# RManLuo/MAMDR

Hardware: AMD Instinct MI355X
Metric: domain-steps/sec (higher is better)
Workload: dtype f32; 1 GPU; mlp_meta_mamdr Taobao-10 bs=1024 (frozen pretrained tables); global_batch=1024, domains=10, step_definition=one MAMDR meta-epoch (DN + DR phases, all outer updates), parallelism=single GPU

## Files before the change

### mamdr_amd/csrc/fused_kernels.hip

```cpp
#include <hip/hip_ext.h>

#include "mamdr_kernels.h"
#include "wgrad_adam_deal.h"

namespace mamdr {

constexpr int FZ_THREADS = 512;
constexpr int FZ_WAVES = 8;
constexpr int FZ_RING = 32;
static_assert(FZ_SBLK == DM_PARTS && FZ_DEAL_EMB == EMB && FZ_DEAL_H1 == H1 && FZ_DEAL_H2 == H2 && FZ_DEAL_H3 == H3,
              "wgrad_adam_deal.h deals the tower of mamdr_device.h");
static_assert(FZ_OUTB == 2 && FZ_OWN == FZ_SBLK + FZ_TILES + FZ_OUTB, "two output-unit workgroups of 32 columns of h3");
__host__ __device__ constexpr int fz_own_wgs(bool with_loss) { return FZ_OWN + (with_loss ? 1 : 0); }
__constant__ const FzDealTable c_fz_deal = fz_deal_table_make();

#define FZSTAMP(k) MAMDR_STAMP(MAMDR_CYCLES, a.stamps && threadIdx.x == 0, a.stamps[blockIdx.x * 8 + (k)])
#define FZREAL(k) MAMDR_STAMP(MAMDR_REALTIME, a.stamps && threadIdx.x == 0, a.stamps[blockIdx.x * 8 + (k)])

__device__ __forceinline__ void fz_store(const FusedArgs& a, int e, float p, float m, float v) {
    if (a.optimizer == 2) {
        a.m[e] = m;
        return;
    }
    if (a.optimizer == 0) {
// ... 111 lines not shown
    return s > FZ_LDS_TILE ? s : FZ_LDS_TILE;
}

__device__ __forceinline__ void fz_tile_body(const FusedArgs& a, const FzTile ft, float* lds) {
    const int tid = threadIdx.x, lane = tid & 63, j = lane & 15, kq = lane >> 4;
    const int w = __builtin_amdgcn_readfirstlane(tid >> 6);
    const int gemm = ft.gemm, ablk = ft.ablk, bblk = ft.bblk;
    const float* A;
    int lda, b_off, dst, ldn;
    if (gemm == 0) {
        A = a.xa + 16 * ablk;
        lda = a.xa_ld;
        b_off = 32 * bblk;
        ldn = H1;
        dst = a.L.w0 + 16 * ablk * H1 + 32 * bblk;
    } else if (gemm == 1) {
        A = a.acts + XDIM + 16 * ablk;
        lda = ACT_LD;
        b_off = H1 + 32 * bblk;
        ldn = H2;
        dst = a.L.w1 + 16 * ablk * H2 + 32 * bblk;
    } else {
        A = a.acts + XDIM + H1 + 16 * ablk;
        lda = ACT_LD;
        b_off = H1 + H2 + 32 * bblk;
        ldn = H3;
        dst = a.L.w2 + 16 * ablk * H3 + 32 * bblk;
    }
    const int em = tid >> 5, en = tid & 31;
    const int e = dst + em * ldn + en;
    const float p0 = a.p[e];
    const float m0 = a.optimizer == 1 ? 0.f : a.m[e];
    const float v0 = a.optimizer == 0 ? a.v[e] : 0.f;
    const bool bias_tile = gemm > 0 && ablk == 0;
    int be = 0;
    float bp0 = 0.f, bm0 = 0.f, bv0 = 0.f;
    if (bias_tile) {
        be = (gemm == 1 ? a.L.b1 + (b_off - H1) : a.L.b2 + (b_off - H1 - H2)) + (tid & 31);
        bp0 = a.p[be];
        bm0 = a.optimizer == 1 ? 0.f : a.m[be];
        bv0 = a.optimizer == 0 ? a.v[be] : 0.f;
    }
    int s0, s1;
    fz_share(a.rows_pad / 4, w, s0, s1);
    f32x4 acc[2] = {(f32x4){0.f, 0.f, 0.f, 0.f}, (f32x4){0.f, 0.f, 0.f, 0.f}};
    f32x2 csum = (f32x2){0.f, 0.f};
    FZSTAMP(1);
    if (bias_tile) fz_dense<true>(A, lda, a.dz + b_off, DZ_LD, s0, s1, acc, csum);
    else fz_dense<false>(A, lda, a.dz + b_off, DZ_LD, s0, s1, acc, csum);
#pragma unroll
    for (int r = 0; r < 4; ++r)
        *reinterpret_cast<f32x2*>(lds + (w * 16 + 4 * kq + r) * 32 + 2 * j) = (f32x2){acc[0][r], acc[1][r]};
    if (bias_tile) {
        csum[0] += __shfl_xor(csum[0], 16);
        csum[1] += __shfl_xor(csum[1], 16);
        csum[0] += __shfl_xor(csum[0], 32);
        csum[1] += __shfl_xor(csum[1], 32);
        if (lane < 16) *reinterpret_cast<f32x2*>(lds + FZ_CS + w * 32 + 2 * j) = csum;
    }
    FZSTAMP(2);
    __syncthreads();
    FZSTAMP(3);
    float g = lds[em * 32 + en];
#pragma unroll
    for (int ww = 1; ww < FZ_WAVES; ++ww) g += lds[(ww * 16 + em) * 32 + en];
    float p = p0, m = m0, v = v0;
    opt_step(a, g, p, m, v);
    fz_store(a, e, p, m, v);
    if (a.wT && a.optimizer != 2) {
        if (gemm == 2 && !(a.flags & FZ_F_W2T_UNREAD)) {
            const int row = (e - a.L.w2) / H3, col = (e - a.L.w2) - row * H3;
            a.wT[W2T_OFF + col * H2 + row] = p;
        } else if (gemm == 1 && !(a.flags & FZ_F_W1T_UNREAD)) {
            const int row = (e - a.L.w1) / H2, col = (e - a.L.w1) - row * H2;
            a.wT[W1T_OFF + col * H1 + row] = p;
        }
    }
    if (bias_tile && tid < 32) {
        float gb_ = lds[FZ_CS + tid];
#pragma unroll
        for (int ww = 1; ww < FZ_WAVES; ++ww) gb_ += lds[FZ_CS + ww * 32 + tid];
        float bp = bp0, bm = bm0, bv = bv0;
        opt_step(a, gb_, bp, bm, bv);
        fz_store(a, be, bp, bm, bv);
    }
    FZSTAMP(4);
}

template <int MT>
__device__ __forceinline__ void fz_s_contract(const FusedArgs& a, int c0, float* lds) {
    const int tid = threadIdx.x, lane = tid & 63, j = lane & 15, kq = lane >> 4;
    const int w = __builtin_amdgcn_readfirstlane(tid >> 6);
    int s0, s1;
    fz_share(a.rows_pad / 4, w, s0, s1);
    f32x4 acc[4];
#pragma unroll
    for (int mt = 0; mt < 4; ++mt) acc[mt] = (f32x4){0.f, 0.f, 0.f, 0.f};
    fz_onehot<MT>(a.domrow, a.dz + c0, DZ_LD, s0, s1, acc);
    if (j < FZ_SC) {
#pragma unroll
        for (int mt = 0; mt < MT; ++mt)
#pragma unroll
            for (int r = 0; r < 4; ++r) lds[(w * (16 * MT) + 16 * mt + 4 * kq + r) * FZ_SC + j] = acc[mt][r];
    }
}

__device__ __forceinline__ void fz_s_body(const FusedArgs& a, int blk, float* lds) {
    const int tid = threadIdx.x;
    const int D = a.n_domain, c0 = FZ_SC * blk;
    const int MT = (D + 15) / 16;
// ... 100 lines not shown

__device__ __forceinline__ void fz_out_body(const FusedArgs& a, int ob, float* lds) {
    const int tid = threadIdx.x, lane = tid & 63, j = lane & 15, kq = lane >> 4;
    const int w = __builtin_amdgcn_readfirstlane(tid >> 6);
    int s0, s1;
    fz_share(a.rows_pad / 4, w, s0, s1);
    const int n = s1 - s0;
    f32x4 acc[2] = {(f32x4){0.f, 0.f, 0.f, 0.f}, (f32x4){0.f, 0.f, 0.f, 0.f}};
    float sg = 0.f;
    FZSTAMP(1);
    if (n > 0) {
        const unsigned aoff = (unsigned)(kq * ACT_LD + 2 * j);
        const float* arow = a.acts + (size_t)(4 * s0) * ACT_LD + XDIM + H1 + H2 + 32 * ob;
        const float* drow = a.dlogit + 4 * s0;
        const int last = n - 1;
        f32x2 ra[FZ_RING];
        float rd[FZ_RING];
#pragma unroll
        for (int u = 0; u < FZ_RING; ++u) {
            const int idx = min(u, last);
            ra[u] = *reinterpret_cast<const f32x2*>(arow + (size_t)idx * 4 * ACT_LD + aoff);
            rd[u] = (drow + idx * 4)[(unsigned)kq];
        }
        __builtin_amdgcn_sched_barrier(0);
        const int passes = (n + FZ_RING - 1) / FZ_RING;
        int base = 0;
        for (int pass = 0; pass + 1 < passes; ++pass, base += FZ_RING) {
#pragma unroll
            for (int u = 0; u < FZ_RING; ++u) {
                const float bv = j == 0 ? rd[u] : 0.f;
                acc[0] = MAMDR_MFMA16(ra[u][0], bv, acc[0]);
                acc[1] = MAMDR_MFMA16(ra[u][1], bv, acc[1]);
                sg += bv;
                const int idx = min(base + u + FZ_RING, last);
                ra[u] = *reinterpret_cast<const f32x2*>(arow + (size_t)idx * 4 * ACT_LD + aoff);
                rd[u] = (drow + idx * 4)[(unsigned)kq];
                __builtin_amdgcn_sched_barrier(0);
            }
        }
#pragma unroll
        for (int u = 0; u < FZ_RING; ++u) {
            const float bv = (j == 0 && base + u < n) ? rd[u] : 0.f;
            acc[0] = MAMDR_MFMA16(ra[u][0], bv, acc[0]);
            acc[1] = MAMDR_MFMA16(ra[u][1], bv, acc[1]);
            sg += bv;
            __builtin_amdgcn_sched_barrier(0);
        }
    }
    if (j == 0) {
#pragma unroll
        for (int r = 0; r < 4; ++r)
            *reinterpret_cast<f32x2*>(lds + w * 32 + 2 * (4 * kq + r)) = (f32x2){acc[0][r], acc[1][r]};
    }
    sg += __shfl_xor(sg, 16);
    sg += __shfl_xor(sg, 32);
    if (lane == 0) lds[256 + w] = sg;
    FZSTAMP(2);
    __syncthreads();
    FZSTAMP(3);
    if (tid < 32) {
        float g = lds[tid];
#pragma unroll
        for (int ww = 1; ww < FZ_WAVES; ++ww) g += lds[ww * 32 + tid];
        const int e = a.L.wo + 32 * ob + tid;
        float p = a.p[e], m = a.optimizer == 1 ? 0.f : a.m[e], v = a.optimizer == 0 ? a.v[e] : 0.f;
        opt_step(a, g, p, m, v);
        fz_store(a, e, p, m, v);
    } else if (tid == 64 && ob == 0) {
        float g = lds[256];
#pragma unroll
        for (int ww = 1; ww < FZ_WAVES; ++ww) g += lds[256 + ww];
        const int e = a.L.gb;
        float p = a.p[e], m = a.optimizer == 1 ? 0.f : a.m[e], v = a.optimizer == 0 ? a.v[e] : 0.f;
        opt_step(a, g, p, m, v);
        fz_store(a, e, p, m, v);
    }
    FZSTAMP(4);
}

__device__ __forceinline__ void fz_loss_body(const FusedArgs& a, float* lds) {
    const int tid = threadIdx.x;
    float ss = 0.f, ls = 0.f;
    for (int e = tid; e < a.n_domain * EMB; e += FZ_THREADS) ss = fmaf(a.p[e], a.p[e], ss);
    for (int e = tid; e < a.n_loss_tiles; e += FZ_THREADS) ls += a.loss_part[e];
    for (int o = 32; o > 0; o >>= 1) {
        ss += __shfl_xor(ss, o);
        ls += __shfl_xor(ls, o);
    }
    if ((tid & 63) == 0) {
        lds[tid >> 6] = ss;
        lds[8 + (tid >> 6)] = ls;
    }
    __syncthreads();
    if (tid == 0) {
        float sst = 0.f, lst = 0.f;
        for (int ww = 0; ww < FZ_WAVES; ++ww) {
            sst += lds[ww];
            lst += lds[8 + ww];
        }
        const float reg = a.l2_emb * a.frozen_sumsq[0] + a.l2_emb * a.frozen_sumsq[1] + a.l2_emb * sst;
        a.loss_out[0] = lst / (float)a.rows + reg;
    }
}

template <typename P>
__device__ __forceinline__ void prep_ids(const P& a, int n_user, int n_item, int64_t pos, int64_t& src, int& u, int& it) {
    src = a.perm ? (int64_t)a.perm[pos] : pos;
    src = src < 0 ? 0 : (src >= a.n_rows_split ? a.n_rows_split - 1 : src);
    u = a.uid[src];
    it = a.pid[src];
    u = u < 0 ? 0 : (u >= n_user ? n_user - 1 : u);
    it = it < 0 ? 0 : (it >= n_item ? n_item - 1 : it);
}
__device__ __forceinline__ const f32x4* prep_src(const float* user_tab, const float* item_tab, int u, int it, int lane) {
    return reinterpret_cast<const f32x4*>(lane < 32 ? user_tab + (size_t)u * EMB + 4 * lane : item_tab + (size_t)it * EMB + 4 * (lane - 32));
}
__device__ __forceinline__ void prep_store_row(float* xpre, int64_t i, int lane, f32x4 v) {
    __builtin_nontemporal_store(v, reinterpret_cast<f32x4*>(xpre + (size_t)i * (2 * EMB) + 4 * lane));
}
template <typename P>
__device__ __forceinline__ void prep_meta(const P& a, int n_domain, int64_t src, int32_t* pdom, float* plabel, int64_t i) {
    const int d = a.dom[src];
    pdom[i] = d < 0 ? 0 : (d >= n_domain ? n_domain - 1 : d);
    plabel[i] = a.label[src];
}
__device__ __forceinline__ void prep_pad_row(float* xpre, int64_t i, int lane) {
    *reinterpret_cast<f32x4*>(xpre + (size_t)i * (2 * EMB) + 4 * lane) = (f32x4){0.f, 0.f, 0.f, 0.f};
}
template <typename P>
__device__ __forceinline__ void prep_pad_meta(const P& a, int32_t* pdom, float* plabel, int64_t i) {
    pdom[i] = a.pad_dom;
    plabel[i] = 0.f;
}

__device__ __forceinline__ int64_t ride_row(const RideArgs& g, int q) {
    if (q < g.seg[0].count) return g.seg[0].out_off + g.seg[0].first + q;
    q -= g.seg[0].count;
    if (q < g.seg[1].count) return g.seg[1].out_off + g.seg[1].first + q;
    return -1;
}
__device__ __forceinline__ void ride_resolve(const RideArgs& g, const RideArgs::Seg& s, int n_domain, int q, int& u, int& it) {
// ... 140 lines not shown
```

### mamdr_amd/csrc/mamdr_kernels.h

```cpp
#pragma once
#include <hip/hip_runtime.h>
#include <hip/hip_ext.h>
#include <stdint.h>

#include "mamdr_device.h"
#include "pregather_plan.h"
#include "host_base.h"

namespace mamdr {

struct OptArgsLite {
    int optimizer;
    float alpha;
    float omb1, omb2, eps;
    float two_l2;
};
constexpr int32_t EMB_UNTOUCHED = 0x7fffffff;

extern thread_local hipEvent_t g_prof_stop;
int env_warn_unknown();
#define MAMDR_LAUNCH(kernel, grid, block, lds, stream, ...)                                               \
    do {                                                                                                  \
        if (::mamdr::g_prof_stop) {                                                                       \
            hipExtLaunchKernelGGL(kernel, grid, block, lds, stream, nullptr, ::mamdr::g_prof_stop, 0, __VA_ARGS__); \
            ::mamdr::g_prof_stop = nullptr;                                                               \
        } else {                                                                                          \
            hipLaunchKernelGGL(kernel, grid, block, lds, stream, __VA_ARGS__);                            \
        }                                                                                                 \
    } while (0)

constexpr int DM_PARTS = 32;
constexpr int DM_PAIRS = DM_PARTS / 2;
struct DmStep {
    const float* snap;
    const float* pdm;
    int n_part, n_domain;
    int optimizer;
    float alpha, omb1, omb2, eps, two_l2;
};
__device__ __forceinline__ f32x4 dm_pair(const DmStep& q, int d, int c4, int j) {
#pragma clang fp contract(off)
    const size_t row = (size_t)d * EMB + 4 * c4, plane = (size_t)q.n_domain * EMB;
    const f32x4 a = *reinterpret_cast<const f32x4*>(q.pdm + (size_t)(2 * j) * plane + row);
    const f32x4 b = *reinterpret_cast<const f32x4*>(q.pdm + (size_t)(2 * j + 1) * plane + row);
    return a + b;
}
__device__ __forceinline__ void dm_load4(const DmStep& q, int d, int c4, f32x4& p, f32x4& m, f32x4& v) {
    const size_t row = (size_t)d * EMB + 4 * c4, plane = (size_t)q.n_domain * EMB;
    p = *reinterpret_cast<const f32x4*>(q.snap + row);
    m = *reinterpret_cast<const f32x4*>(q.snap + plane + row);
    v = *reinterpret_cast<const f32x4*>(q.snap + 2 * plane + row);
}
__device__ __forceinline__ void dm_apply4(const DmStep& q, f32x4 g, f32x4& p, f32x4& m, f32x4& v) {
#pragma clang fp contract(off)
#pragma unroll
    for (int k = 0; k < 4; ++k) {
        const float gk = g[k] + q.two_l2 * p[k];
        if (q.optimizer == 0) {
// ... 162 lines not shown
    } else {
        m = m + gk;
    }
}
struct DmWave {
    float r[8], w[8];
    float rp, rm, rv, wp, wm, wv;
};
struct DmWaveAddr {
    const float* rb;
    const float* wb;
    const float* rs;
    const float* ws;
};
__device__ __forceinline__ void dm_wave_addr(const TowerArgs& a, int tile, DmWaveAddr& q) {
    const int lane = (int)threadIdx.x & 63, l = lane & 15, gq = lane >> 4, c = 16 * ((int)threadIdx.x >> 6) + l;
    const size_t plane = (size_t)a.n_domain * EMB;
    const size_t er = (size_t)a.dm_hint * EMB + c, ew = (size_t)min(tile, a.n_domain - 1) * EMB + c;
    q.rb = a.dms.pdm + (size_t)(8 * gq) * plane + er;
    q.wb = a.dms.pdm + (size_t)(8 * gq) * plane + ew;
    q.rs = a.dms.snap + er;
    q.ws = (a.dms.snap ? a.dms.snap : a.dm_live_p) + ew;
}
__device__ __forceinline__ void dm_wave_begin(const TowerArgs& a, int tile, bool do_read, const DmWaveAddr& q, DmWave& t) {
    const bool pend = a.dms.snap != nullptr, wr = tile < a.n_domain;
    const size_t plane = (size_t)a.n_domain * EMB;
#pragma unroll
    for (int k = 0; k < 8; ++k) t.r[k] = t.w[k] = 0.f;
    t.rp = t.rm = t.rv = t.wp = t.wm = t.wv = 0.f;
    if (pend && do_read) {
#pragma unroll
        for (int k = 0; k < 8; ++k) t.r[k] = q.rb[(size_t)k * plane];
        t.rp = q.rs[0];
        t.rm = q.rs[plane];
        t.rv = q.rs[2 * plane];
    }
    if (wr) {
        if (pend) {
#pragma unroll
            for (int k = 0; k < 8; ++k) t.w[k] = q.wb[(size_t)k * plane];
            t.wp = q.ws[0];
            t.wm = q.ws[plane];
            t.wv = q.ws[2 * plane];
        } else {
            const size_t off = (size_t)(q.ws - a.dm_live_p);
            t.wp = q.ws[0];
            t.wm = a.dm_live_m[off];
            t.wv = a.dm_live_v[off];
        }
    }
}
__device__ __forceinline__ float dm_wave_sum(const float (&x)[8]) {
#pragma clang fp contract(off)
    const int l = (int)threadIdx.x & 15;
    const float G = (((x[0] + x[1]) + (x[2] + x[3])) + (x[4] + x[5])) + (x[6] + x[7]);
    const float G0 = __shfl(G, l), G1 = __shfl(G, l + 16), G2 = __shfl(G, l + 32), G3 = __shfl(G, l + 48);
    return ((G0 + G1) + G2) + G3;
}
__device__ __forceinline__ void dm_elem_finish(const DmStep& q, int c, const float* parts, float& p, float& m, float& v) {
#pragma clang fp contract(off)
    float t[DM_PAIRS];
#pragma unroll
    for (int j = 0; j < DM_PAIRS; ++j) t[j] = parts[j * EMB + c];
    float G[4];
#pragma unroll
    for (int gq = 0; gq < 4; ++gq) G[gq] = ((t[4 * gq] + t[4 * gq + 1]) + t[4 * gq + 2]) + t[4 * gq + 3];
    dm_apply1(q, ((G[0] + G[1]) + G[2]) + G[3], p, m, v);
}
struct DmTile {
    f32x4 pr[2][2], pw[2][2];
    float p, m, v;
};
__device__ __forceinline__ void dm_pair_load(const DmStep& q, int d, int c4, int j, f32x4 (&t)[2]) {
    const size_t row = (size_t)d * EMB + 4 * c4, plane = (size_t)q.n_domain * EMB;
    t[0] = *reinterpret_cast<const f32x4*>(q.pdm + (size_t)(2 * j) * plane + row);
    t[1] = *reinterpret_cast<const f32x4*>(q.pdm + (size_t)(2 * j + 1) * plane + row);
}
__device__ __forceinline__ f32x4 dm_pair_add(const f32x4 (&t)[2]) {
#pragma clang fp contract(off)
    return t[0] + t[1];
}
__device__ __forceinline__ void dm_tile_begin(const TowerArgs& a, int tile, int d_read, DmTile& t) {
    const int wv = __builtin_amdgcn_readfirstlane((int)threadIdx.x >> 6);
    const f32x4 zero = (f32x4){0.f, 0.f, 0.f, 0.f};
    t.pr[0][0] = t.pr[0][1] = t.pr[1][0] = t.pr[1][1] = zero;
    t.pw[0][0] = t.pw[0][1] = t.pw[1][0] = t.pw[1][1] = zero;
    t.p = t.m = t.v = 0.f;
    if (wv < 4) return;
    const bool pend = a.dms.snap != nullptr, wr = tile < a.n_domain;
    const int dw = min(tile, a.n_domain - 1);
    const int lp = (int)threadIdx.x - 256, grp = lp >> 5, c4 = lp & 31;
    if (pend) {
        dm_pair_load(a.dms, d_read, c4, grp, t.pr[0]);
        dm_pair_load(a.dms, d_read, c4, grp + 8, t.pr[1]);
        if (wr) {
            dm_pair_load(a.dms, dw, c4, grp, t.pw[0]);
            dm_pair_load(a.dms, dw, c4, grp + 8, t.pw[1]);
        }
    }
    const size_t plane = (size_t)a.n_domain * EMB;
    const int c = lp & (EMB - 1);
    if (wv < 6) {
        if (pend) {
            const size_t e = (size_t)d_read * EMB + c;
            t.p = a.dms.snap[e];
            t.m = a.dms.snap[plane + e];
            t.v = a.dms.snap[2 * plane + e];
        }
    } else if (wr) {
        const size_t e = (size_t)dw * EMB + c;
// ... 672 lines not shown
```

### mamdr_amd/csrc/tower4_kernels.hip

```cpp
#include <hip/hip_ext.h>

#include <cstdint>
#include <cstdio>
#include <cstdlib>

#include "mamdr_kernels.h"

namespace mamdr {

constexpr int T4_ROWS = 4;
constexpr int T4_THREADS = 512;
constexpr int T4_WAVES = 8;
constexpr int T4_PF = 8;
constexpr int T4_DEEP = 8;

constexpr int T4_XLD = XDIM + 4, T4_H1LD = H1 + 4, T4_H2LD = H2 + 4, T4_H3LD = H3 + 4;
constexpr int T4_XS = 0;
constexpr int T4_H1 = T4_XS + T4_ROWS * T4_XLD;
constexpr int T4_H2 = T4_H1 + T4_ROWS * T4_H1LD;
constexpr int T4_DZ3 = T4_H2 + T4_ROWS * T4_H2LD;
constexpr int T4_DZ2 = T4_H2;
constexpr int T4_DZ1 = T4_H1;
constexpr int T4_RED = T4_DZ3 + T4_ROWS * T4_H3LD;
constexpr int T4_RED_FLOATS = 4 * T4_ROWS * H1;
// ... 140 lines not shown
        return W + (size_t)((threadIdx.x >> 6) * 32) * H1 + 4 * (threadIdx.x & 63);
    }
    static __device__ __forceinline__ const float* wptr2(const float* __restrict__ W) {
        return W + (size_t)(2 * EMB + (threadIdx.x >> 6) * 16) * H1 + 4 * (threadIdx.x & 63);
    }
    __device__ __forceinline__ void prefetch(const float* __restrict__ W, bool skip1 = false) {
        const float* wp = skip1 ? wptr2(W) : wptr1(W);
#pragma unroll
        for (int u = 0; u < T4_PF; ++u) t4_load<4>(b[u], wp + (size_t)u * H1);
        __builtin_amdgcn_sched_barrier(0);
    }
};
template <typename MidSeg, typename Mid>
__device__ __forceinline__ void t4_contract_l0(T4L0& tw, const float* __restrict__ W, const float* xs, float* red,
                                               f32x4 (&acc)[4], MidSeg midseg, Mid mid, bool skip1 = false) {
    static_assert(T4_PF == 8, "two segments of 32 and 16 rows, 8-deep ring");
    const int lane = threadIdx.x & 63, w = threadIdx.x >> 6;
    const float* wp1 = T4L0::wptr1(W);
    const float* wp2 = T4L0::wptr2(W);
    const float* ap1 = xs + (lane & 3) * T4_XLD + 32 * w;
    const float* ap2 = xs + (lane & 3) * T4_XLD + 2 * EMB + 16 * w;
    auto chunk = [&](const float* ap, const float* next, bool reload) {
#pragma unroll
        for (int q = 0; q < T4_PF; q += 4) {
            const f32x4 a4 = *reinterpret_cast<const f32x4*>(ap + q);
            __builtin_amdgcn_sched_barrier(0);
#pragma unroll
            for (int u = 0; u < 4; ++u) {
#pragma unroll
                for (int t = 0; t < 4; ++t) acc[t] = MAMDR_MFMA4(a4[u], tw.b[q + u][t], acc[t]);
                if (reload) t4_load<4>(tw.b[q + u], next + (size_t)(q + u) * H1);
            }
            __builtin_amdgcn_sched_barrier(0);
        }
    };
    if (!skip1) {
#pragma unroll 1
        for (int k0 = 0; k0 < 24; k0 += 8) chunk(ap1 + k0, wp1 + (size_t)(k0 + 8) * H1, true);
        chunk(ap1 + 24, wp2, true);
    }
    midseg();
    chunk(ap2, wp2 + (size_t)8 * H1, true);
    chunk(ap2 + 8, wp2, false);
    mid();
    t4_put<H1, 4, false>(acc, red);
}

template <int ROWS>
__device__ __forceinline__ void t4_w1_request(const float* __restrict__ W1, float* w1s, const int row0) {
    w1_image_request<ROWS>(W1, w1s, row0);
}
__device__ __forceinline__ void t4_w1_landed() { w1_image_landed(); }

template <typename Mid>
__device__ __forceinline__ void t4_contract_w1f(const float* w1s, const float* As, float* red, Mid mid) {
    const int lane = threadIdx.x & 63, w = threadIdx.x >> 6;
    const float* ap = As + (lane & 3) * T4_H1LD + 32 * w;
    const float* wp = w1s + (32 * w) * H2 + 2 * (lane & 1);
    const int half = lane >> 1;
    f32x4 acc[2];
    acc[0] = acc[1] = (f32x4){0.f, 0.f, 0.f, 0.f};
    f32x2 b[2][8];
    f32x4 a4[2][2];
    auto request = [&](int c, int buf) {
#pragma unroll
        for (int u = 0; u < 8; ++u) {
            const int k = 8 * c + u;
            b[buf][u] = *reinterpret_cast<const f32x2*>(wp + k * H2 + 4 * (half ^ k));
        }
        a4[buf][0] = *reinterpret_cast<const f32x4*>(ap + 8 * c);
        a4[buf][1] = *reinterpret_cast<const f32x4*>(ap + 8 * c + 4);
    };
    request(0, 0);
#pragma unroll
    for (int c = 0; c < 4; ++c) {
        const int cur = c & 1;
        __builtin_amdgcn_sched_barrier(0);
        if (c + 1 < 4) request(c + 1, cur ^ 1);
        __builtin_amdgcn_sched_barrier(0);
#pragma unroll
        for (int u = 0; u < 8; ++u) {
            acc[0] = MAMDR_MFMA4(a4[cur][u >> 2][u & 3], b[cur][u][0], acc[0]);
            acc[1] = MAMDR_MFMA4(a4[cur][u >> 2][u & 3], b[cur][u][1], acc[1]);
        }
    }
    mid();
    t4_put<H2, 2, false>(acc, red);
}
template <typename Mid>
__device__ __forceinline__ void t4_contract_w1b(const float* w1s, const float* As, float* red, Mid mid) {
    const int lane = threadIdx.x & 63, w = threadIdx.x >> 6;
    const float* ap = As + (lane & 3) * T4_H2LD + 16 * w;
    const float* rp = w1s + lane * H2;
    const int sw = lane & 31;
    f32x4 acc[4];
#pragma unroll
    for (int t = 0; t < 4; ++t) acc[t] = (f32x4){0.f, 0.f, 0.f, 0.f};
    f32x4 b[2][4], a4[2];
    auto request = [&](int c, int buf) {
        const int pos = 4 * ((4 * w + c) ^ sw);
#pragma unroll
        for (int t = 0; t < 4; ++t) b[buf][t] = *reinterpret_cast<const f32x4*>(rp + t * 64 * H2 + pos);
        a4[buf] = *reinterpret_cast<const f32x4*>(ap + 4 * c);
    };
    request(0, 0);
#pragma unroll
    for (int c = 0; c < 4; ++c) {
        const int cur = c & 1;
        __builtin_amdgcn_sched_barrier(0);
        if (c + 1 < 4) request(c + 1, cur ^ 1);
        __builtin_amdgcn_sched_barrier(0);
#pragma unroll
        for (int j = 0; j < 4; ++j)
#pragma unroll
            for (int t = 0; t < 4; ++t) acc[t] = MAMDR_MFMA4(a4[cur][j], b[cur][t][j], acc[t]);
    }
    mid();
    t4_put<H1, 4, true>(acc, red);
}

template <int N>
__device__ __forceinline__ float t4_sum(const float* red, int row, int col) {
    constexpr int SLOTS = N > H2 ? 4 : T4_WAVES;
    float s = red[row * N + col];
#pragma unroll
    for (int w = 1; w < SLOTS; ++w) s += red[(w * T4_ROWS + row) * N + col];
    return s;
}

#define T4STAMP(k) MAMDR_STAMP(MAMDR_CYCLES, a.stamps && threadIdx.x == 0, a.stamps[blockIdx.x * 16 + (k)])
#define T4STAMP_W4(k) MAMDR_STAMP(MAMDR_CYCLES, a.stamps && threadIdx.x == 256, a.stamps[(blockIdx.x + 256) * 16 + (k)])
#define T4REAL(k) MAMDR_STAMP(MAMDR_REALTIME, a.stamps && threadIdx.x == 0, a.stamps[blockIdx.x * 16 + (k)])

template <bool DX, bool FM, bool W1L, bool PRE = false, bool W2D = false>
__global__ __launch_bounds__(T4_THREADS) void k_tower4(const float* __restrict__ k_xpre, const int32_t* __restrict__ k_pdom,
                                                       const float* __restrict__ k_plabel, const float* __restrict__ k_w0,
                                                       const float* __restrict__ k_w1, const int k_rows, const TowerArgs a) {
    static_assert(!PRE || (!DX && !FM), "pre-gathered passes serve the frozen-table mlp tower");
    static_assert(!W2D || (PRE && W1L), "W2 read in place: the W1-image instance of the pre-gathered tower");
    extern __shared__ __attribute__((aligned(16))) float smem[];
    const int tid = threadIdx.x, lane = tid & 63, w = tid >> 6;
    const int tile = blockIdx.x;
    const int n_tiles = (int)gridDim.x;
    const int r0 = tile * T4_ROWS;
    int* rowi = reinterpret_cast<int*>(smem + T4_ROWI);
    float* rowf = smem + T4_ROWI + 16;
    float* red = smem + T4_RED;
    const float* P = a.dense;
    float* acts_t = a.acts + (size_t)r0 * ACT_LD;
    float* dz_t = a.dz + (size_t)r0 * DZ_LD;

    T4L0 w0;
    T4W<H1, H2, T4_DEEP> w1;
    T4W<H2, H3, W1L ? 16 : T4_DEEP> w2;
    T4W<H3, H2> v2;
    T4W<H2, H1, T4_DEEP> v1;
    float* w1s = smem + T4_W1S;
    T4W<H1, 2 * EMB> v0;
    f32x4 acc0[4];
#pragma unroll
    for (int t = 0; t < 4; ++t) acc0[t] = (f32x4){0.f, 0.f, 0.f, 0.f};
    asm volatile("" : "+v"(acc0[0]), "+v"(acc0[1]), "+v"(acc0[2]), "+v"(acc0[3]));
    T4REAL(10);
    T4STAMP(0);
    int perm_src = 0;
    constexpr bool FUSED_OK = !DX && !FM;
    constexpr bool pre = PRE;
    f32x4 xv = (f32x4){0.f, 0.f, 0.f, 0.f};
    int pre_dom = 0;
    float pre_lab = 0.f;
    if (pre) {
        const int rr = min(r0 + ((lane >> 3) & 3), max(k_rows - 1, 0));
        xv = *reinterpret_cast<const f32x4*>(k_xpre + (size_t)rr * (2 * EMB) + 32 * w + 4 * (lane & 7));
        const int rb = min(r0 + (tid & 3), max(k_rows - 1, 0));
        pre_dom = k_pdom[rb];
        pre_lab = k_plabel[rb];
    } else if (a.perm) {
        const int64_t pc = a.row_base + min(r0 + (tid & (T4_ROWS - 1)), max(a.rows - 1, 0));
        perm_src = a.perm[pc];
    }
    __builtin_amdgcn_sched_barrier(0);
    const bool l0_dom_only = FM && a.deepfm == 4;
    w0.prefetch(k_w0, l0_dom_only);
    const bool dmw = FUSED_OK && a.dm_snap_out != nullptr;
    DmWave dmt;
    DmWaveAddr dma;
    if (dmw) dm_wave_addr(a, tile, dma);
    const int ecol = tid & 255, erow2 = tid >> 8;
    const float b0r = P[a.L.b0 + ecol];
    const float b1r = P[a.L.b1 + (tid & 127)];
    const float b2r = P[a.L.b2 + (tid & 63)];
    const float wor = P[a.L.wo + (tid & 63)];
    const float gbr = P[a.L.gb];
    __builtin_amdgcn_sched_barrier(0);
    if (W1L && pre) t4_w1_request<32>(k_w1, w1s, 32 * __builtin_amdgcn_readfirstlane(w));
    __builtin_amdgcn_sched_barrier(0);

    if (pre) {
        const int row = (lane >> 3) & 3;
        if (r0 + row >= a.rows) xv = (f32x4){0.f, 0.f, 0.f, 0.f};
        *reinterpret_cast<f32x4*>(smem + T4_XS + row * T4_XLD + 32 * w + 4 * (lane & 7)) = xv;
        __builtin_amdgcn_fence(__ATOMIC_RELEASE, "wavefront");
        __builtin_amdgcn_wave_barrier();
        __builtin_amdgcn_fence(__ATOMIC_ACQUIRE, "wavefront");
        if (tid < T4_ROWS) {
            const bool valid = (r0 + tid) < a.rows;
            rowi[tid] = 0;
            rowi[4 + tid] = 0;
            rowi[8 + tid] = pre_dom;
            rowi[12 + tid] = valid ? 1 : 0;
// ... 99 lines not shown
            rowf[48 + tid] = v;
            a.ipbuf[(size_t)(r0 + r) * 4 + j] = v;
            if (j == 0) rowf[8 + r] = 0.f;
        }
    }

    T4STAMP(1);
    const float scale = a.use_dropout ? a.keep_scale : 1.0f;
    const bool drop = a.use_dropout != 0;

    t4_contract_l0(w0, k_w0, smem + T4_XS, red, acc0,
                   [&]() {
                       if (!dmw) return;
                       T4STAMP(13);
                       const int c = 16 * w + (lane & 15);
                       if (same) {
                           float p = dmt.rp, m = dmt.rm, v = dmt.rv;
                           dm_apply1(a.dms, dm_wave_sum(dmt.r), p, m, v);
                           if (lane < 16) {
#pragma unroll
                               for (int rr = 0; rr < T4_ROWS; ++rr) smem[T4_XS + rr * T4_XLD + 2 * EMB + c] = r0 + rr < a.rows ? p : 0.f;
                           }
                       }
                       T4STAMP(14);
                       if (tile < a.n_domain) {
                           float p = dmt.wp, m = dmt.wm, v = dmt.wv;
                           if (pend) dm_apply1(a.dms, dm_wave_sum(dmt.w), p, m, v);
                           if (lane < 16) dm_store_elem(a, (size_t)tile * EMB + c, pend, p, m, v);
                       }
                       if (tile + n_tiles < a.n_domain && tid < EMB / 4) {
                           for (int d = tile + n_tiles; d < a.n_domain; d += n_tiles) {
                               f32x4 p4, m4, v4;
                               const size_t row = (size_t)d * EMB + 4 * tid, plane = (size_t)a.n_domain * EMB;
                               if (pend) {
                                   dm_step4(a.dms, d, tid, p4, m4, v4);
                                   if (a.dms.optimizer != 2) *reinterpret_cast<f32x4*>(a.dm_live_p + row) = p4;
                                   if (a.dms.optimizer != 1) *reinterpret_cast<f32x4*>(a.dm_live_m + row) = m4;
                                   if (a.dms.optimizer == 0) *reinterpret_cast<f32x4*>(a.dm_live_v + row) = v4;
                               } else {
                                   p4 = *reinterpret_cast<const f32x4*>(a.dm_live_p + row);
                                   m4 = *reinterpret_cast<const f32x4*>(a.dm_live_m + row);
                                   v4 = *reinterpret_cast<const f32x4*>(a.dm_live_v + row);
                               }
                               *reinterpret_cast<f32x4*>(a.dm_snap_out + row) = p4;
                               *reinterpret_cast<f32x4*>(a.dm_snap_out + plane + row) = m4;
                               *reinterpret_cast<f32x4*>(a.dm_snap_out + 2 * plane + row) = v4;
                           }
                       }
                       T4STAMP(15);
                   },
                   [&]() {
                       if (W1L) {
                           t4_w1_landed();
                           w2.prefetch(P + a.L.w2);
                       } else {
                           w1.prefetch(P + a.L.w1);
                       }
                   },
                   l0_dom_only);
    T4STAMP(2);
    if (!pre && tid < T4_ROWS * (XDIM / 4)) {
        const int row = tid / (XDIM / 4), c4 = tid - row * (XDIM / 4);
        *reinterpret_cast<f32x4*>(acts_t + (size_t)row * ACT_LD + c4 * 4) =
            *reinterpret_cast<const f32x4*>(smem + T4_XS + row * T4_XLD + c4 * 4);
    }
    __syncthreads();
    {
        const uint32_t key = dropout_layer_key(a.seed, a.step, 0);
#pragma unroll
        for (int rr = 0; rr < 2; ++rr) {
            const int row = erow2 + 2 * rr;
            float z = t4_sum<H1>(red, row, ecol) + b0r;
            if (pnn) z += (rowf[48 + 4 * row] * wx0 + rowf[49 + 4 * row] * wx1) + rowf[50 + 4 * row] * wx2;
            float h = fmaxf(z, 0.f);
            if (drop) {
                const uint32_t u = mamdr_dropout_u32(key, (uint32_t)(r0 + row) * (uint32_t)H1 + (uint32_t)ecol);
                h = (u >= a.drop_thresh) ? h * scale : 0.f;
            }
            smem[T4_H1 + row * T4_H1LD + ecol] = h;
            ws_store1(&acts_t[(size_t)row * ACT_LD + XDIM + ecol], h);
        }
    }
    __syncthreads();

    T4STAMP(3);
    if (W1L) t4_contract_w1f(w1s, smem + T4_H1, red, [&]() {
        if constexpr (W2D) v2.prefetch_untransposed(P + a.L.w2);
        else v2.prefetch(a.wT + W2T_OFF);
    });
    else t4_contract(w1, P + a.L.w1, smem + T4_H1, T4_H1LD, red, [&]() { w2.prefetch(P + a.L.w2); });
    __syncthreads();
    T4STAMP(4);
    {
        const uint32_t key = dropout_layer_key(a.seed, a.step, 1);
        const int row = tid >> 7, col = tid & 127;
        float h = fmaxf(t4_sum<H2>(red, row, col) + b1r, 0.f);
        if (drop) {
            const uint32_t u = mamdr_dropout_u32(key, (uint32_t)(r0 + row) * (uint32_t)H2 + (uint32_t)col);
            h = (u >= a.drop_thresh) ? h * scale : 0.f;
        }
        smem[T4_H2 + row * T4_H2LD + col] = h;
        ws_store1(&acts_t[(size_t)row * ACT_LD + XDIM + H1 + col], h);
    }
    __syncthreads();

    T4STAMP(5);
    t4_contract(w2, P + a.L.w2, smem + T4_H2, T4_H2LD, red, [&]() {
        if (!W1L) {
            v2.prefetch(a.wT + W2T_OFF);
            v1.prefetch(a.wT + W1T_OFF);
        } else if (DX) {
            v0.prefetch(a.wT + W0T_OFF);
        }
    });
    __syncthreads();
    T4STAMP(6);
    if (w < T4_ROWS) {
        const uint32_t key = dropout_layer_key(a.seed, a.step, 2);
        const int row = w, col = lane;
        float h = fmaxf(t4_sum<H3>(red, row, col) + b2r, 0.f);
        if (drop) {
            const uint32_t u = mamdr_dropout_u32(key, (uint32_t)(r0 + row) * (uint32_t)H3 + (uint32_t)col);
            h = (u >= a.drop_thresh) ? h * scale : 0.f;
        }
        ws_store1(&acts_t[(size_t)row * ACT_LD + XDIM + H1 + H2 + col], h);
        float s = h * wor;
        for (int o = 32; o > 0; o >>= 1) s += __shfl_xor(s, o);
        float logit = s + gbr;
        if (FM) logit += rowf[8 + row];
        float p;
        if (logit >= 0.f) {
            p = 1.0f / (1.0f + __expf(-logit));
        } else {
            const float ez = __expf(logit);
            p = ez / (1.0f + ez);
        }
        const bool valid = rowi[12 + row] != 0;
        const float y = rowf[row];
        const float lo = 1e-7f, hi = 1.0f - 1e-7f;
        const float pc = fminf(fmaxf(p, lo), hi);
        const float zc = __logf(pc / (1.0f - pc));
        const float loss = fmaxf(zc, 0.f) - zc * y + __logf(1.0f + __expf(-fabsf(zc)));
        const float inside = (p >= lo && p <= hi) ? 1.0f : 0.0f;
        float dl = valid ? ((p - y) * inside) / (float)a.rows : 0.0f;
        if (a.uw_off >= 0) {
            const float var = P[a.uw_off];
            dl *= 1.0f / (var * var);
        }
        if (lane == 0) {
            a.dlogit[r0 + row] = dl;
            a.domrow[r0 + row] = rowi[8 + row];
            rowf[4 + row] = valid ? loss : 0.f;
            rowf[12 + row] = dl;
            if (DX) {
                a.urow[r0 + row] = valid ? rowi[row] : -1;
                a.irow[r0 + row] = valid ? rowi[4 + row] : -1;
                if (valid && a.map_u) {
                    atomicMin(a.map_u + rowi[row], r0 + row);
                    atomicMin(a.map_i + rowi[4 + row], r0 + row);
                }
            }
        }
        const float d = (h > 0.f) ? (dl * wor) * scale : 0.f;
        smem[T4_DZ3 + row * T4_H3LD + col] = d;
        ws_store1(&dz_t[(size_t)row * DZ_LD + H1 + H2 + col], d);
    }
    __syncthreads();
    if (tid == 0) a.loss_part[tile] = (rowf[4] + rowf[5]) + (rowf[6] + rowf[7]);
    if (FM && !pnn && !nfm) {
        const int row = tid >> 7, k = tid & 127;
        const float* xr = smem + T4_XS + row * T4_XLD;
        a.fmq[(size_t)(r0 + row) * EMB + k] = a.deepfm == 1 ? rowf[12 + row] * (xr[k] + xr[EMB + k]) : 0.f;
    }

    T4STAMP(7);
    t4_contract(v2, a.wT + W2T_OFF, smem + T4_DZ3, T4_H3LD, red, []() {});
    __syncthreads();
    {
        const int row = tid >> 7, col = tid & 127;
        const float v = t4_sum<H2>(red, row, col);
        const float d = (smem[T4_H2 + row * T4_H2LD + col] > 0.f) ? v * scale : 0.f;
        smem[T4_DZ2 + row * T4_H2LD + col] = d;
        ws_store1(&dz_t[(size_t)row * DZ_LD + H1 + col], d);
    }
    __syncthreads();
    T4STAMP(8);
    if (W1L) t4_contract_w1b(w1s, smem + T4_DZ2, red, []() {});
    else t4_contract(v1, a.wT + W1T_OFF, smem + T4_DZ2, T4_H2LD, red, [&]() { if (DX) v0.prefetch(a.wT + W0T_OFF); });
    __syncthreads();
    float dip[2][3] = {{0.f, 0.f, 0.f}, {0.f, 0.f, 0.f}};
#pragma unroll
    for (int rr = 0; rr < 2; ++rr) {
        const int row = erow2 + 2 * rr;
        const float v = t4_sum<H1>(red, row, ecol);
        const float d = (smem[T4_H1 + row * T4_H1LD + ecol] > 0.f) ? v * scale : 0.f;
        ws_store1(&dz_t[(size_t)row * DZ_LD + ecol], d);
        if (DX || nfm) smem[T4_DZ1 + row * T4_H1LD + ecol] = d;
        dip[rr][0] = d * wx0;
        dip[rr][1] = d * wx1;
        dip[rr][2] = d * wx2;
    }
    T4STAMP(9);
    T4REAL(11);
    if (pnn) {
#pragma unroll
        for (int rr = 0; rr < 2; ++rr)
#pragma unroll
            for (int j = 0; j < 3; ++j)
                for (int o = 32; o > 0; o >>= 1) dip[rr][j] += __shfl_xor(dip[rr][j], o);
        __syncthreads();
        if (lane == 0) {
#pragma unroll
            for (int rr = 0; rr < 2; ++rr)
#pragma unroll
                for (int j = 0; j < 3; ++j) red[(w * 2 + rr) * 4 + j] = dip[rr][j];
        }
        __syncthreads();
        if (tid < 4 * T4_ROWS) {
            const int r = tid >> 2, j = tid & 3;
            float v = 0.f;
            if (j < 3) {
                const int w0_ = 4 * (r & 1), rr = r >> 1;
                v = ((red[((w0_ + 0) * 2 + rr) * 4 + j] + red[((w0_ + 1) * 2 + rr) * 4 + j]) + red[((w0_ + 2) * 2 + rr) * 4 + j]) +
                    red[((w0_ + 3) * 2 + rr) * 4 + j];
            }
            rowf[64 + tid] = v;
        }
        __syncthreads();
        {
            const int row = tid >> 7, k = tid & 127;
            const float* xr = smem + T4_XS + row * T4_XLD;
            a.fmq[(size_t)(r0 + row) * EMB + k] = rowf[65 + 4 * row] * xr[k] + rowf[66 + 4 * row] * xr[EMB + k];
        }
    }
    if (nfm) {
        __syncthreads();
        {
            const float* wn = P + a.L.w0 + (size_t)(2 * EMB + 2 * lane) * H1 + 32 * w;
            const float* ap = smem + T4_DZ1 + (lane & 3) * T4_H1LD + 32 * w;
            f32x4 acc[2];
// ... 133 lines not shown
```

Before: 47870 domain-steps/s.

## Use DPP/permlane wave reductions and hoist W1 LDS loads ahead of barriers

Replaces __shfl_xor-based wave reductions and row gathers with DPP and gfx950 permlane16/32 swap intrinsics, so cross-lane reductions avoid LDS-backed ds_bpermute traffic. Separately, the W1 forward and backward tile fragments are now loaded from LDS into registers earlier (forward in the prefetch callback, backward before a barrier), letting their latency overlap other work before the MFMA contraction. This raises register pressure because full W1 fragments (T4W1F, T4W1B) stay live across phases, which may reduce occupancy or cause spills. It also adds timestamp hooks at the first MFMA.

```diff
diff --git a/mamdr_amd/csrc/fused_kernels.hip b/mamdr_amd/csrc/fused_kernels.hip
--- a/mamdr_amd/csrc/fused_kernels.hip
+++ b/mamdr_amd/csrc/fused_kernels.hip
@@ -187,10 +187,8 @@
     for (int r = 0; r < 4; ++r)
         *reinterpret_cast<f32x2*>(lds + (w * 16 + 4 * kq + r) * 32 + 2 * j) = (f32x2){acc[0][r], acc[1][r]};
     if (bias_tile) {
-        csum[0] += __shfl_xor(csum[0], 16);
-        csum[1] += __shfl_xor(csum[1], 16);
-        csum[0] += __shfl_xor(csum[0], 32);
-        csum[1] += __shfl_xor(csum[1], 32);
+        csum[0] = wave_xor_sum_16_32(csum[0]);
+        csum[1] = wave_xor_sum_16_32(csum[1]);
         if (lane < 16) *reinterpret_cast<f32x2*>(lds + FZ_CS + w * 32 + 2 * j) = csum;
     }
     FZSTAMP(2);
@@ -397,8 +395,7 @@
         for (int r = 0; r < 4; ++r)
             *reinterpret_cast<f32x2*>(lds + w * 32 + 2 * (4 * kq + r)) = (f32x2){acc[0][r], acc[1][r]};
     }
-    sg += __shfl_xor(sg, 16);
-    sg += __shfl_xor(sg, 32);
+    sg = wave_xor_sum_16_32(sg);
     if (lane == 0) lds[256 + w] = sg;
     FZSTAMP(2);
     __syncthreads();
@@ -428,10 +425,8 @@
     float ss = 0.f, ls = 0.f;
     for (int e = tid; e < a.n_domain * EMB; e += FZ_THREADS) ss = fmaf(a.p[e], a.p[e], ss);
     for (int e = tid; e < a.n_loss_tiles; e += FZ_THREADS) ls += a.loss_part[e];
-    for (int o = 32; o > 0; o >>= 1) {
-        ss += __shfl_xor(ss, o);
-        ls += __shfl_xor(ls, o);
-    }
+    ss = wave_xor_sum64(ss);
+    ls = wave_xor_sum64(ls);
     if ((tid & 63) == 0) {
         lds[tid >> 6] = ss;
         lds[8 + (tid >> 6)] = ls;
diff --git a/mamdr_amd/csrc/mamdr_kernels.h b/mamdr_amd/csrc/mamdr_kernels.h
--- a/mamdr_amd/csrc/mamdr_kernels.h
+++ b/mamdr_amd/csrc/mamdr_kernels.h
@@ -4,6 +4,7 @@
 #include <stdint.h>
 
 #include "mamdr_device.h"
+#include "wave_exchange.h"
 #include "pregather_plan.h"
 #include "host_base.h"
 
@@ -272,10 +273,10 @@
 }
 __device__ __forceinline__ float dm_wave_sum(const float (&x)[8]) {
 #pragma clang fp contract(off)
-    const int l = (int)threadIdx.x & 15;
     const float G = (((x[0] + x[1]) + (x[2] + x[3])) + (x[4] + x[5])) + (x[6] + x[7]);
-    const float G0 = __shfl(G, l), G1 = __shfl(G, l + 16), G2 = __shfl(G, l + 32), G3 = __shfl(G, l + 48);
-    return ((G0 + G1) + G2) + G3;
+    float Gq[4];
+    wave_gather_rows16(G, Gq);
+    return ((Gq[0] + Gq[1]) + Gq[2]) + Gq[3];
 }
 __device__ __forceinline__ void dm_elem_finish(const DmStep& q, int c, const float* parts, float& p, float& m, float& v) {
 #pragma clang fp contract(off)
diff --git a/mamdr_amd/csrc/tower4_kernels.hip b/mamdr_amd/csrc/tower4_kernels.hip
--- a/mamdr_amd/csrc/tower4_kernels.hip
+++ b/mamdr_amd/csrc/tower4_kernels.hip
@@ -216,26 +216,46 @@
 }
 __device__ __forceinline__ void t4_w1_landed() { w1_image_landed(); }
 
-template <typename Mid>
-__device__ __forceinline__ void t4_contract_w1f(const float* w1s, const float* As, float* red, Mid mid) {
+struct T4W1F {
+    f32x2 b[32];
+};
+struct T4W1B {
+    f32x4 b[4][4];
+};
+__device__ __forceinline__ void t4_w1f_request(const float* w1s, T4W1F& q) {
+    const int lane = threadIdx.x & 63, w = threadIdx.x >> 6;
+    const float* wp = w1s + (32 * w) * H2 + 2 * (lane & 1);
+    const int half = lane >> 1;
+#pragma unroll
+    for (int k = 0; k < 32; ++k)
+        q.b[k] = *reinterpret_cast<const f32x2*>(wp + k * H2 + 4 * (half ^ k));
+    __builtin_amdgcn_sched_barrier(0);
+}
+__device__ __forceinline__ void t4_w1b_request(const float* w1s, T4W1B& q) {
+    const int lane = threadIdx.x & 63, w = threadIdx.x >> 6;
+    const float* rp = w1s + lane * H2;
+    const int sw = lane & 31;
+#pragma unroll
+    for (int c = 0; c < 4; ++c) {
+        const int pos = 4 * ((4 * w + c) ^ sw);
+#pragma unroll
+        for (int t = 0; t < 4; ++t) q.b[c][t] = *reinterpret_cast<const f32x4*>(rp + t * 64 * H2 + pos);
+    }
+    __builtin_amdgcn_sched_barrier(0);
+}
+template <typename Stamp, typename Mid>
+__device__ __forceinline__ void t4_contract_w1f(const T4W1F& q, const float* As, float* red, Stamp first_mfma, Mid mid) {
     const int lane = threadIdx.x & 63, w = threadIdx.x >> 6;
     const float* ap = As + (lane & 3) * T4_H1LD + 32 * w;
-    const float* wp = w1s + (32 * w) * H2 + 2 * (lane & 1);
-    const int half = lane >> 1;
     f32x4 acc[2];
     acc[0] = acc[1] = (f32x4){0.f, 0.f, 0.f, 0.f};
-    f32x2 b[2][8];
     f32x4 a4[2][2];
     auto request = [&](int c, int buf) {
-#pragma unroll
-        for (int u = 0; u < 8; ++u) {
-            const int k = 8 * c + u;
-            b[buf][u] = *reinterpret_cast<const f32x2*>(wp + k * H2 + 4 * (half ^ k));
-        }
         a4[buf][0] = *reinterpret_cast<const f32x4*>(ap + 8 * c);
         a4[buf][1] = *reinterpret_cast<const f32x4*>(ap + 8 * c + 4);
     };
     request(0, 0);
+    first_mfma();
 #pragma unroll
     for (int c = 0; c < 4; ++c) {
         const int cur = c & 1;
@@ -244,40 +264,33 @@
         __builtin_amdgcn_sched_barrier(0);
 #pragma unroll
         for (int u = 0; u < 8; ++u) {
-            acc[0] = MAMDR_MFMA4(a4[cur][u >> 2][u & 3], b[cur][u][0], acc[0]);
-            acc[1] = MAMDR_MFMA4(a4[cur][u >> 2][u & 3], b[cur][u][1], acc[1]);
+            acc[0] = MAMDR_MFMA4(a4[cur][u >> 2][u & 3], q.b[8 * c + u][0], acc[0]);
+            acc[1] = MAMDR_MFMA4(a4[cur][u >> 2][u & 3], q.b[8 * c + u][1], acc[1]);
         }
     }
     mid();
     t4_put<H2, 2, false>(acc, red);
 }
-template <typename Mid>
-__device__ __forceinline__ void t4_contract_w1b(const float* w1s, const float* As, float* red, Mid mid) {
+template <typename Stamp, typename Mid>
+__device__ __forceinline__ void t4_contract_w1b(const T4W1B& q, const float* As, float* red, Stamp first_mfma, Mid mid) {
     const int lane = threadIdx.x & 63, w = threadIdx.x >> 6;
     const float* ap = As + (lane & 3) * T4_H2LD + 16 * w;
-    const float* rp = w1s + lane * H2;
-    const int sw = lane & 31;
     f32x4 acc[4];
 #pragma unroll
     for (int t = 0; t < 4; ++t) acc[t] = (f32x4){0.f, 0.f, 0.f, 0.f};
-    f32x4 b[2][4], a4[2];
-    auto request = [&](int c, int buf) {
-        const int pos = 4 * ((4 * w + c) ^ sw);
-#pragma unroll
-        for (int t = 0; t < 4; ++t) b[buf][t] = *reinterpret_cast<const f32x4*>(rp + t * 64 * H2 + pos);
-        a4[buf] = *reinterpret_cast<const f32x4*>(ap + 4 * c);
-    };
-    request(0, 0);
+    f32x4 a4[2];
+    a4[0] = *reinterpret_cast<const f32x4*>(ap);
+    first_mfma();
 #pragma unroll
     for (int c = 0; c < 4; ++c) {
         const int cur = c & 1;
         __builtin_amdgcn_sched_barrier(0);
-        if (c + 1 < 4) request(c + 1, cur ^ 1);
+        if (c + 1 < 4) a4[cur ^ 1] = *reinterpret_cast<const f32x4*>(ap + 4 * (c + 1));
         __builtin_amdgcn_sched_barrier(0);
 #pragma unroll
         for (int j = 0; j < 4; ++j)
 #pragma unroll
-            for (int t = 0; t < 4; ++t) acc[t] = MAMDR_MFMA4(a4[cur][j], b[cur][t][j], acc[t]);
+            for (int t = 0; t < 4; ++t) acc[t] = MAMDR_MFMA4(a4[cur][j], q.b[c][t][j], acc[t]);
     }
     mid();
     t4_put<H1, 4, true>(acc, red);
@@ -294,6 +307,7 @@
 
 #define T4STAMP(k) MAMDR_STAMP(MAMDR_CYCLES, a.stamps && threadIdx.x == 0, a.stamps[blockIdx.x * 16 + (k)])
 #define T4STAMP_W4(k) MAMDR_STAMP(MAMDR_CYCLES, a.stamps && threadIdx.x == 256, a.stamps[(blockIdx.x + 256) * 16 + (k)])
+#define T4STAMP_X(k) MAMDR_STAMP(MAMDR_CYCLES, a.stamps && threadIdx.x == 0, a.stamps[(blockIdx.x + 256) * 16 + 8 + (k)])
 #define T4REAL(k) MAMDR_STAMP(MAMDR_REALTIME, a.stamps && threadIdx.x == 0, a.stamps[blockIdx.x * 16 + (k)])
 
 template <bool DX, bool FM, bool W1L, bool PRE = false, bool W2D = false>
@@ -320,6 +334,8 @@
     T4W<H3, H2> v2;
     T4W<H2, H1, T4_DEEP> v1;
     float* w1s = smem + T4_W1S;
+    T4W1F w1f;
+    T4W1B w1b;
     T4W<H1, 2 * EMB> v0;
     f32x4 acc0[4];
 #pragma unroll
@@ -525,6 +541,7 @@
                    [&]() {
                        if (W1L) {
                            t4_w1_landed();
+                           t4_w1f_request(w1s, w1f);
                            w2.prefetch(P + a.L.w2);
                        } else {
                            w1.prefetch(P + a.L.w1);
@@ -557,7 +574,7 @@
     __syncthreads();
 
     T4STAMP(3);
-    if (W1L) t4_contract_w1f(w1s, smem + T4_H1, red, [&]() {
+    if (W1L) t4_contract_w1f(w1f, smem + T4_H1, red, [&]() { T4STAMP_X(0); }, [&]() {
         if constexpr (W2D) v2.prefetch_untransposed(P + a.L.w2);
         else v2.prefetch(a.wT + W2T_OFF);
     });
@@ -597,8 +614,7 @@
             h = (u >= a.drop_thresh) ? h * scale : 0.f;
         }
         ws_store1(&acts_t[(size_t)row * ACT_LD + XDIM + H1 + H2 + col], h);
-        float s = h * wor;
-        for (int o = 32; o > 0; o >>= 1) s += __shfl_xor(s, o);
+        const float s = wave_xor_dot64(h, wor);
         float logit = s + gbr;
         if (FM) logit += rowf[8 + row];
         float p;
@@ -638,6 +654,7 @@
         smem[T4_DZ3 + row * T4_H3LD + col] = d;
         ws_store1(&dz_t[(size_t)row * DZ_LD + H1 + H2 + col], d);
     }
+    if (W1L) t4_w1b_request(w1s, w1b);
     __syncthreads();
     if (tid == 0) a.loss_part[tile] = (rowf[4] + rowf[5]) + (rowf[6] + rowf[7]);
     if (FM && !pnn && !nfm) {
@@ -658,7 +675,7 @@
     }
     __syncthreads();
     T4STAMP(8);
-    if (W1L) t4_contract_w1b(w1s, smem + T4_DZ2, red, []() {});
+    if (W1L) t4_contract_w1b(w1b, smem + T4_DZ2, red, [&]() { T4STAMP_X(1); }, []() {});
     else t4_contract(v1, a.wT + W1T_OFF, smem + T4_DZ2, T4_H2LD, red, [&]() { if (DX) v0.prefetch(a.wT + W0T_OFF); });
     __syncthreads();
     float dip[2][3] = {{0.f, 0.f, 0.f}, {0.f, 0.f, 0.f}};
diff --git a/mamdr_amd/csrc/wave_exchange.h b/mamdr_amd/csrc/wave_exchange.h
--- /dev/null
+++ b/mamdr_amd/csrc/wave_exchange.h
@@ -0,0 +1,105 @@
+#pragma once
+#include <hip/hip_runtime.h>
+
+namespace mamdr {
+
+template <int CTRL, int BANKS>
+__device__ __forceinline__ float wave_dpp_mov(float old, float x) {
+    return __builtin_bit_cast(float, __builtin_amdgcn_update_dpp(__builtin_bit_cast(int, old), __builtin_bit_cast(int, x), CTRL,
+                                                                 0xf, BANKS, false));
+}
+struct WaveSwap {
+    float a, b;
+};
+template <int O>
+__device__ __forceinline__ WaveSwap wave_swap(float x, float y) {
+    static_assert(O == 16 || O == 32, "the two swaps of gfx950");
+    const unsigned ux = __builtin_bit_cast(unsigned, x), uy = __builtin_bit_cast(unsigned, y);
+    const auto r = O == 32 ? __builtin_amdgcn_permlane32_swap(ux, uy, false, false)
+                           : __builtin_amdgcn_permlane16_swap(ux, uy, false, false);
+    const unsigned a = r[0], b = r[1];
+    return WaveSwap{__builtin_bit_cast(float, a), __builtin_bit_cast(float, b)};
+}
+template <int O>
+__device__ __forceinline__ float wave_xor_get(float x) {
+    static_assert(O == 1 || O == 2 || O == 4 || O == 8 || O == 16 || O == 32, "one butterfly step of a 64-lane wave");
+    if constexpr (O == 32 || O == 16) {
+        const WaveSwap r = wave_swap<O>(x, x);
+        return ((threadIdx.x & 63) & O) != 0 ? r.a : r.b;
+    } else if constexpr (O == 8) {
+        return wave_dpp_mov<0x128, 0xf>(x, x);
+    } else if constexpr (O == 4) {
+        const float up = wave_dpp_mov<0x104, 0x5>(x, x);
+        return wave_dpp_mov<0x114, 0xa>(up, x);
+    } else if constexpr (O == 2) {
+        return wave_dpp_mov<0x4e, 0xf>(x, x);
+    } else {
+        return wave_dpp_mov<0xb1, 0xf>(x, x);
+    }
+}
+template <int O>
+__device__ __forceinline__ float wave_xor_get_ref(float x) { return __shfl_xor(x, O); }
+
+template <int O>
+__device__ __forceinline__ float wave_xor_add(float x) {
+    if constexpr (O == 32 || O == 16) {
+        const WaveSwap r = wave_swap<O>(x, x);
+        return r.a + r.b;
+    } else {
+        return x + wave_xor_get<O>(x);
+    }
+}
+template <int O>
+__device__ __forceinline__ float wave_xor_add_ref(float x) { return x + __shfl_xor(x, O); }
+
+__device__ __forceinline__ float wave_xor_sum64(float s) {
+    s = wave_xor_add<32>(s);
+    s = wave_xor_add<16>(s);
+    s = wave_xor_add<8>(s);
+    s = wave_xor_add<4>(s);
+    s = wave_xor_add<2>(s);
+    s = wave_xor_add<1>(s);
+    return s;
+}
+__device__ __forceinline__ float wave_xor_sum64_ref(float s) {
+    for (int o = 32; o > 0; o >>= 1) s += __shfl_xor(s, o);
+    return s;
+}
+
+__device__ __forceinline__ float wave_xor_dot64(float a, float b) {
+    float s = __builtin_fmaf(a, b, wave_xor_get<32>(a * b));
+    s = wave_xor_add<16>(s);
+    s = wave_xor_add<8>(s);
+    s = wave_xor_add<4>(s);
+    s = wave_xor_add<2>(s);
+    s = wave_xor_add<1>(s);
+    return s;
+}
+__device__ __forceinline__ float wave_xor_dot64_ref(float a, float b) {
+    float s = __builtin_fmaf(a, b, __shfl_xor(a * b, 32));
+    for (int o = 16; o > 0; o >>= 1) s += __shfl_xor(s, o);
+    return s;
+}
+
+__device__ __forceinline__ float wave_xor_sum_16_32(float s) { return wave_xor_add<32>(wave_xor_add<16>(s)); }
+__device__ __forceinline__ float wave_xor_sum_16_32_ref(float s) {
+    s += __shfl_xor(s, 16);
+    s += __shfl_xor(s, 32);
+    return s;
+}
+
+__device__ __forceinline__ void wave_gather_rows16(float x, float (&g)[4]) {
+    const WaveSwap r = wave_swap<16>(x, x);
+    const WaveSwap e = wave_swap<32>(r.a, r.a), o = wave_swap<32>(r.b, r.b);
+    g[0] = e.a;
+    g[1] = o.a;
+    g[2] = e.b;
+    g[3] = o.b;
+}
+__device__ __forceinline__ void wave_gather_rows16_ref(float x, float (&g)[4]) {
+    const int l = (int)threadIdx.x & 15;
+#pragma unroll
+    for (int q = 0; q < 4; ++q) g[q] = __shfl(x, l + 16 * q);
+}
+
+}
```

After: 48410 domain-steps/s, median of 6. 1.01x the previous value.
